# argsim/argsim

Hardware: AMD Instinct MI355X
Metric: sentences/sec per ELBO step (higher is better)
Workload: dtype f32; 1 GPU; BASELINE configs[1]: 1xMI355X fp32, latent_dim 128, vocab 8k, seq_len 64, batch 256 per GPU; FULL synthetic Zipf batches, dim_emb 512, 3 layers, step 20000; global_batch=256, seq_len=64, parallelism=dp1, gru=persistent

## Files before the change

### argsim_amd/csrc/gemm_f32.hip

```cpp
#include "kernels.h"
#include "mfma_tile.h"
#include <algorithm>
#include <cstdlib>
#include <type_traits>

namespace avae {

constexpr int BK = kTileBK, LDK = kTileLDK;

template <bool XC, int ROWS>
struct FastTile {
    const float* base; long long step, valid; unsigned voff[ROWS / 32];
    __device__ __forceinline__ void init(const float* P, int ld, int x0, int X, int kb, int ke, int tid)
    {
        if (XC) {
            base = P + (size_t)kb * ld + x0; step = (long long)BK * ld; valid = (long long)(ke - kb) * ld - x0;
#pragma unroll
            for (int rep = 0; rep < ROWS / 32; ++rep) { const int f = tid + 256 * rep; voff[rep] = (unsigned)(((f / (ROWS / 4)) * ld + ((f % (ROWS / 4)) << 2)) * 4); }
        } else {
            base = P + (size_t)x0 * ld + kb; step = BK; valid = (long long)(X - x0) * ld - kb;
#pragma unroll
            for (int rep = 0; rep < ROWS / 32; ++rep) { const int f = tid + 256 * rep; voff[rep] = (unsigned)(((f >> 3) * ld + ((f & 7) << 2)) * 4); }
        }
    }
    __device__ __forceinline__ void load(float4 (&r)[ROWS / 32], int it) const
    {
        const long long rem = valid - it * step;
        const unsigned bytes = rem <= 0 ? 0u : (rem >= (1ll << 30) ? 0xFFFFFFFFu : (unsigned)(rem * 4));
        const __amdgpu_buffer_rsrc_t rs = __builtin_amdgcn_make_buffer_rsrc(const_cast<float*>(base + it * step), 0, (int)bytes, 0x00020000);
#pragma unroll
        for (int rep = 0; rep < ROWS / 32; ++rep) {
            const u32x4 v = __builtin_amdgcn_raw_buffer_load_b128(rs, (int)voff[rep], 0, 0);
            r[rep] = make_float4(__uint_as_float(v.x), __uint_as_float(v.y), __uint_as_float(v.z), __uint_as_float(v.w));
        }
    }
};

template <int MODE>
__device__ __forceinline__ void put(float* c, float v)
{
    if (MODE == 2) atomicAdd(c, v);
    else if (MODE == 1) *c += v;
    else *c = v;
}
template <int TM, int TN, int WN, int MODE>
__device__ __forceinline__ void epilogue_full(const GemmArgs& g, const f32x16 (&acc)[TM][TN], int m0, int n0, int wm, int wn, int h, int l31, bool add_bias)
{
    float bv[TN];
#pragma unroll
    for (int j = 0; j < TN; ++j) bv[j] = add_bias ? g.bias[n0 + 32 * (wn * TN + j) + l31] : 0.f;
#pragma unroll
    for (int j = 0; j < TN; ++j) {
        const int col = n0 + 32 * (wn * TN + j) + l31;
#pragma unroll
        for (int i = 0; i < TM; ++i) {
            float* c = g.C + (size_t)(m0 + 32 * (wm * TM + i) + 4 * h) * g.ldc + col;
#pragma unroll
            for (int r = 0; r < 16; ++r)
                put<MODE>(c + (size_t)mfma32_row(r, 0) * g.ldc, g.alpha * acc[i][j][r] + bv[j]);
        }
    }
}
template <int TM, int TN, int WN>
__device__ __forceinline__ void epilogue(const GemmArgs& g, const f32x16 (&acc)[TM][TN], int M, int m0, int n0, int BM, int BN,
                                         int wm, int wn, int h, int l31, bool atomic, bool add_bias)
{
    if (!atomic && m0 + BM <= M && n0 + BN <= g.N) {
        if (g.accumulate) epilogue_full<TM, TN, WN, 1>(g, acc, m0, n0, wm, wn, h, l31, add_bias);
        else epilogue_full<TM, TN, WN, 0>(g, acc, m0, n0, wm, wn, h, l31, add_bias);
        return;
    }
    epilogue_generic<TM, TN>(acc, g.C, g.ldc, M, g.N, m0 + 32 * wm * TM, n0 + 32 * wn * TN, h, l31, g.alpha, add_bias ? g.bias : nullptr,
                             atomic ? kEpiAtomic : (g.accumulate ? kEpiAccumulate : kEpiStore));
}

template <bool A_MC, bool B_NC, int WM, int WN, int TM, int TN, bool FAST = false, bool DB = false>
__global__ __launch_bounds__(256, DB ? 2 : 3) void gemm_f32_kernel(GemmArgs g)
{
    constexpr int BM = 32 * WM * TM, BN = 32 * WN * TN;
    constexpr int kStage = (BM + BN) * LDK;
    __shared__ __attribute__((aligned(16))) float smem[kStage * (DB ? 2 : 1)];
    float* As = smem;
    float* Bs = smem + BM * LDK;

    const int tid = threadIdx.x, lane = tid & 63, wave = tid >> 6;
    const int h = lane >> 5, l31 = lane & 31;
    const int wm = wave / WN, wn = wave % WN;

    if (blockIdx.y) { g.A = g.A2; g.B = g.B2; g.C = g.C2; g.bias = g.bias2; }
    int M = g.M, K = g.K;
    if (g.dyn_kind == 1) M = min(M, *g.dyn);
    if (g.dyn_kind == 2) K = min(K, *g.dyn);

    const int tiles_n = (g.N + BN - 1) / BN;
    const int nblk = ((M + BM - 1) / BM) * tiles_n;
    const int bid = xcd_tile(blockIdx.x, nblk);
    if (bid < 0) return;
    const int tm = bid / tiles_n, tn = bid - tm * tiles_n;
    const int m0 = tm * BM, n0 = tn * BN;
    if (m0 >= M) return;

    int kb = 0, ke = K;
    if (g.split_k > 1) {
        int ktiles = (K + BK - 1) / BK;
        int per = (ktiles + g.split_k - 1) / g.split_k;
        kb = blockIdx.z * per * BK;
        ke = min(K, kb + per * BK);
        if (kb >= ke) return;
    }

    f32x16 acc[TM][TN];
    zero_acc(acc);

    float4 ra[BM / 32], rb[BN / 32];
    FastTile<A_MC, BM> fa; FastTile<B_NC, BN> fb;
    if (FAST) {
        fa.init(g.A, g.lda, m0, M, kb, ke, tid); fb.init(g.B, g.ldb, n0, g.N, kb, ke, tid);
        fa.load(ra, 0); fb.load(rb, 0);
    } else {
        load_tile<A_MC, BM>(ra, g.A, g.lda, m0, M, kb, ke, tid);
        load_tile<B_NC, BN>(rb, g.B, g.ldb, n0, g.N, kb, ke, tid);
    }

    if (DB) {
        store_tile<A_MC, BM>(As, ra, tid);
        store_tile<B_NC, BN>(Bs, rb, tid);
        __syncthreads();
    }
    for (int k0 = kb; k0 < ke; k0 += BK) {
        auto next_loads = [&]() __attribute__((always_inline)) {
            if (k0 + BK < ke) {
                if (FAST) { const int it = (k0 - kb) / BK + 1; fa.load(ra, it); fb.load(rb, it); }
                else {
                    load_tile<A_MC, BM>(ra, g.A, g.lda, m0, M, k0 + BK, ke, tid);
                    load_tile<B_NC, BN>(rb, g.B, g.ldb, n0, g.N, k0 + BK, ke, tid);
                }
            }
        };
        if (!DB) {
            store_tile<A_MC, BM>(As, ra, tid);
            store_tile<B_NC, BN>(Bs, rb, tid);
            next_loads();
            __syncthreads();
        } else next_loads();
        __builtin_amdgcn_s_setprio(1);
#pragma unroll
        for (int q = 0; q < 4; ++q) {
            float a[TM][4], b[TN][4];
#pragma unroll
            for (int t = 0; t < TM; ++t) {
                if (A_MC) {
#pragma unroll
                    for (int e = 0; e < 4; ++e) a[t][e] = As[(8 * q + 4 * h + e) * BM + 32 * (wm * TM + t) + l31];
                } else {
                    float4 v = *reinterpret_cast<const float4*>(As + (32 * (wm * TM + t) + l31) * LDK + 8 * q + 4 * h);
                    a[t][0] = v.x; a[t][1] = v.y; a[t][2] = v.z; a[t][3] = v.w;
                }
            }
#pragma unroll
            for (int t = 0; t < TN; ++t) {
                if (B_NC) {
#pragma unroll
                    for (int e = 0; e < 4; ++e) b[t][e] = Bs[(8 * q + 4 * h + e) * BN + 32 * (wn * TN + t) + l31];
                } else {
                    float4 v = *reinterpret_cast<const float4*>(Bs + (32 * (wn * TN + t) + l31) * LDK + 8 * q + 4 * h);
                    b[t][0] = v.x; b[t][1] = v.y; b[t][2] = v.z; b[t][3] = v.w;
                }
            }
#pragma unroll
            for (int e = 0; e < 4; ++e)
#pragma unroll
                for (int i = 0; i < TM; ++i)
#pragma unroll
                    for (int j = 0; j < TN; ++j)
                        acc[i][j] = __builtin_amdgcn_mfma_f32_32x32x2f32(a[i][e], b[j][e], acc[i][j], 0, 0, 0);
        }
        __builtin_amdgcn_s_setprio(0);
        if (DB) {
            As = (As == smem) ? smem + kStage : smem;
            Bs = As + BM * LDK;
            if (k0 + BK < ke) {
                store_tile<A_MC, BM>(As, ra, tid);
                store_tile<B_NC, BN>(Bs, rb, tid);
            }
        }
        __syncthreads();
    }

    const bool atomic = g.split_k > 1;
    const bool add_bias = g.bias != nullptr && (!atomic || blockIdx.z == 0);
    epilogue<TM, TN, WN>(g, acc, M, m0, n0, BM, BN, wm, wn, h, l31, atomic, add_bias);
}

template <bool A_MC, bool B_NC, bool FAST>
__global__ __launch_bounds__(256, 3) void gemm_f32_persist_kernel(GemmArgs g)
{
    static_assert(FAST, "buffer-load staging only (register budget of three workgroups per CU)");
    constexpr int TM = 2, TN = 2, WN = 2, BM = 128, BN = 128;
    __shared__ __attribute__((aligned(16))) float smem[(BM + BN) * LDK];
    float* As = smem;
    float* Bs = smem + BM * LDK;
    const int tid = threadIdx.x, lane = tid & 63, wave = tid >> 6;
    const int h = lane >> 5, l31 = lane & 31;
    const int wm = wave / WN, wn = wave % WN;

    int M = g.M;
    const int K = g.K;
    if (g.dyn_kind == 1) M = min(M, *g.dyn);
    const int tiles_n = (g.N + BN - 1) / BN;
    const int nblk = ((M + BM - 1) / BM) * tiles_n;
    const int per_xcd = gridDim.x >> 3;
    int run0, run_n;
    xcd_run(blockIdx.x & 7, nblk, run0, run_n);
    int local = blockIdx.x >> 3;
    if (local >= run_n) return;

    float4 ra[BM / 32], rb[BN / 32];
    FastTile<A_MC, BM> fa; FastTile<B_NC, BN> fb;
    auto first_tile = [&](int bid) __attribute__((always_inline)) {
        const int tm = bid / tiles_n, tn = bid - tm * tiles_n;
        if (FAST) {
            fa.init(g.A, g.lda, tm * BM, M, 0, K, tid); fb.init(g.B, g.ldb, tn * BN, g.N, 0, K, tid);
            fa.load(ra, 0); fb.load(rb, 0);
        } else {
            load_tile<A_MC, BM>(ra, g.A, g.lda, tm * BM, M, 0, K, tid);
            load_tile<B_NC, BN>(rb, g.B, g.ldb, tn * BN, g.N, 0, K, tid);
        }
    };
    first_tile(run0 + local);
    for (; local < run_n; local += per_xcd) {
        const int bid = run0 + local;
        const int tm = bid / tiles_n, tn = bid - tm * tiles_n;
        const int m0 = tm * BM, n0 = tn * BN;
        const bool more = local + per_xcd < run_n;
        f32x16 acc[TM][TN];
        zero_acc(acc);
        for (int k0 = 0; k0 < K; k0 += BK) {
            store_tile<A_MC, BM>(As, ra, tid);
            store_tile<B_NC, BN>(Bs, rb, tid);
// ... 45 lines not shown
                } else b[u] = *reinterpret_cast<const float4*>(bp + k);
            }
        }
#pragma unroll
        for (int u = 0; u < 4; ++u) {
            if (kk + 8 * u >= k1) break;
            acc = __builtin_amdgcn_mfma_f32_32x32x2f32(a[u].x, b[u].x, acc, 0, 0, 0);
            acc = __builtin_amdgcn_mfma_f32_32x32x2f32(a[u].y, b[u].y, acc, 0, 0, 0);
            acc = __builtin_amdgcn_mfma_f32_32x32x2f32(a[u].z, b[u].z, acc, 0, 0, 0);
            acc = __builtin_amdgcn_mfma_f32_32x32x2f32(a[u].w, b[u].w, acc, 0, 0, 0);
        }
    }
    if (wave > 0) {
#pragma unroll
        for (int r = 0; r < 16; ++r) red[wave - 1][r][lane] = acc[r];
    }
    __syncthreads();
    if (wave > 0) return;
    const int col = n0 + l31;
    if (col >= g.N) return;
    const float bv = g.bias ? g.bias[col] : 0.f;
#pragma unroll
    for (int r = 0; r < 16; ++r) {
        float v = acc[r];
#pragma unroll
        for (int w = 0; w < 7; ++w) v += red[w][r][lane];
        const int row = m0 + mfma32_row(r, h);
        if (row >= g.M) continue;
        float* c = g.C + (size_t)row * g.ldc + col;
        v = g.alpha * v + bv;
        if (g.accumulate) *c += v; else *c = v;
    }
}
static bool skinny_ok(bool a_mc, const GemmArgs& g)
{
    return !a_mc && g.split_k <= 1 && g.dyn_kind == 0 && (g.K & 3) == 0 && (g.lda & 3) == 0 && g.K >= 64;
}
static void launch_skinny(hipStream_t st, bool b_nc, const GemmArgs& g, const GemmF32Form& f)
{
    const dim3 grid(f.gx, f.gy, f.gz);
    if (b_nc) hipLaunchKernelGGL(gemm_f32_skinny_kernel<true>, grid, dim3(512), 0, st, g);
    else      hipLaunchKernelGGL(gemm_f32_skinny_kernel<false>, grid, dim3(512), 0, st, g);
}

template <class F>
static void with_layouts(bool a_mc, bool b_nc, F&& f)
{
    if (!a_mc && !b_nc)      f(std::false_type{}, std::false_type{});
    else if (!a_mc && b_nc)  f(std::false_type{}, std::true_type{});
    else if (a_mc && b_nc)   f(std::true_type{}, std::true_type{});
    else                     f(std::true_type{}, std::false_type{});
}

GemmF32Form gemm_f32_form(bool a_mc, bool b_nc, const GemmArgs& g)
{
    GemmF32Form f{-1, false, false, false, 0, 0, 0, hipSuccess};
    if (g.M <= 0 || g.N <= 0) return f;
    f.err = hipErrorInvalidValue;
    if ((g.lda | g.ldb) & 3) return f;
    if (((uintptr_t)g.A | (uintptr_t)g.B | (uintptr_t)g.A2 | (uintptr_t)g.B2) & 15) return f;
    if (!a_mc && (g.K & 3)) return f;
    if (a_mc && (g.M & 3)) return f;
    if (!b_nc && (g.K & 3)) return f;
    if (b_nc && (g.N & 3)) return f;
    if (g.dyn_kind == 2 && (!a_mc || !b_nc || (g.split_k > 1 && g.bias))) return f;
    f.err = hipSuccess;
    if (g.thin == 3 && skinny_ok(a_mc, g) && (b_nc || (g.ldb & 3) == 0)) {
        f.tile = 3; f.gx = ((g.M + 31) / 32) * ((g.N + 31) / 32); f.gy = g.A2 ? 2 : 1; f.gz = 1;
        return f;
    }
    f.tile = g.thin == 2 ? 2 : (g.thin ? 1 : 0);
    const int BM = f.tile == 0 ? 128 : (f.tile == 1 ? 32 : 64), BN = f.tile == 2 ? 64 : 128;
    const int tiles = ((g.M + BM - 1) / BM) * ((g.N + BN - 1) / BN);
    f.gx = tiles; f.gy = g.A2 ? 2 : 1; f.gz = g.split_k > 1 ? g.split_k : 1;
    static const bool allow_fast = !getenv("AVAE_F32_NOFAST");
    const int k_per_wg = g.split_k > 1 ? (g.K + g.split_k - 1) / g.split_k : g.K;
    f.fast = allow_fast && (a_mc ? (g.M % BM == 0) : (g.K % BK == 0 && g.dyn_kind != 2)) &&
             (b_nc ? (g.N % BN == 0) : (g.K % BK == 0 && g.dyn_kind != 2)) && (a_mc || b_nc || k_per_wg >= 1536);
    if (f.tile == 1) return f;
    static const char* ps_env = getenv("AVAE_F32_PERSIST");
    const bool aligned = (a_mc ? (g.M % BM == 0) : (g.K % BK == 0)) && (b_nc ? (g.N % BN == 0) : (g.K % BK == 0));
    const bool persist = (ps_env ? atoi(ps_env) != 0 : true) && allow_fast && aligned && !g.A2 && g.split_k <= 1 && g.dyn_kind != 2 && tiles > 1024;
    if (persist) {
        f.tile = 0; f.fast = true; f.persist = true; f.gx = 768; f.gy = f.gz = 1;
        return f;
    }
    static const char* db_env = getenv("AVAE_F32_DB");
    const int eff_tiles = (g.dyn_kind == 1 && g.dyn_expect > 0) ? std::min(tiles, ((g.dyn_expect + BM - 1) / BM) * ((g.N + BN - 1) / BN)) : (g.dyn_kind == 1 ? 0 : tiles);
    f.db = db_env ? atoi(db_env) != 0 && !g.A2 : (!g.A2 && g.split_k <= 1 && eff_tiles > 768 && tiles <= 1024);
    return f;
}

template <int WM, int WN, int TM, int TN>
static void launch_variant(hipStream_t st, bool a_mc, bool b_nc, const GemmArgs& g, const GemmF32Form& f)
{
    const dim3 grid(f.gx, f.gy, f.gz);
    if constexpr (WM == 2 && WN == 2) {
        if (f.persist) {
            with_layouts(a_mc, b_nc, [&](auto A, auto B) { hipLaunchKernelGGL((gemm_f32_persist_kernel<decltype(A)::value, decltype(B)::value, true>), grid, dim3(256), 0, st, g); });
            return;
        }
        if (f.db) {
            if (f.fast) {
                with_layouts(a_mc, b_nc, [&](auto A, auto B) { hipLaunchKernelGGL((gemm_f32_kernel<decltype(A)::value, decltype(B)::value, WM, WN, TM, TN, true, true>), grid, dim3(256), 0, st, g); });
            } else {
                with_layouts(a_mc, b_nc, [&](auto A, auto B) { hipLaunchKernelGGL((gemm_f32_kernel<decltype(A)::value, decltype(B)::value, WM, WN, TM, TN, false, true>), grid, dim3(256), 0, st, g); });
            }
            return;
        }
    }
    if (f.fast) {
        with_layouts(a_mc, b_nc, [&](auto A, auto B) { hipLaunchKernelGGL((gemm_f32_kernel<decltype(A)::value, decltype(B)::value, WM, WN, TM, TN, true>), grid, dim3(256), 0, st, g); });
        return;
    }
    with_layouts(a_mc, b_nc, [&](auto A, auto B) { hipLaunchKernelGGL((gemm_f32_kernel<decltype(A)::value, decltype(B)::value, WM, WN, TM, TN>), grid, dim3(256), 0, st, g); });
}

hipError_t gemm_f32(hipStream_t st, bool a_mc, bool b_nc, const GemmArgs& g)
{
    const GemmF32Form f = gemm_f32_form(a_mc, b_nc, g);
    if (f.err != hipSuccess) return f.err;
    if (f.tile < 0) return hipSuccess;
    if (f.tile == 3) launch_skinny(st, b_nc, g, f);
    else if (f.persist) launch_variant<2, 2, 2, 2>(st, a_mc, b_nc, g, f);
    else if (f.tile == 2) launch_variant<2, 2, 1, 1>(st, a_mc, b_nc, g, f);
    else if (f.tile == 1) launch_variant<1, 4, 1, 1>(st, a_mc, b_nc, g, f);
    else launch_variant<2, 2, 2, 2>(st, a_mc, b_nc, g, f);
    return hipGetLastError();
}

}
```

### argsim_amd/csrc/handle.cpp

```cpp
#include "ctx.h"

using namespace avae;
using namespace avae::host;

static std::string g_create_err;

namespace avae { namespace host {

int grow_scratch(avae_ctx* h, size_t need, const char* what)
{
    if (h->scratch_n >= (int64_t)need) return 0;
    AV_CHECK(hipStreamSynchronize(h->stream));
    if (h->scratch) AV_CHECK(hipFree(h->scratch));
    h->scratch = nullptr; h->scratch_n = 0;
    if (hipMalloc(reinterpret_cast<void**>(&h->scratch), need) != hipSuccess) {
        (void)hipGetLastError();
        h->scratch = nullptr;
        char b_[256]; snprintf(b_, sizeof b_, "%s: %.0f MB of scratch could not be allocated on the device", what, (double)need / 1048576.0);
        return fail(h, b_);
    }
    h->scratch_n = (int64_t)need;
    return 0;
}

// ... 178 lines not shown
    if (shape) for (int i = 0; i < 4; ++i) shape[i] = e->shape[i];
    return 0;
}

static int xfer_tensor(avae_handle h, const char* name, int kind, float* buf, bool get)
{
    if (!h) return 1;
    AV_TRY(check_bound(h));
    const ParamEntry* e = find_param(h, name);
    if (!e) return fail(h, std::string("unknown variable: ") + (name ? name : "(null)"));
    float* base = state_buf(h, kind);
    if (!base) return fail(h, "bad tensor kind");
    float* flat = base + e->offset;
    int64_t n = e->shape[0] * e->shape[1] * e->shape[2] * e->shape[3];
    if (!e->g16) {
        AV_CHECK(hipMemcpyAsync(get ? buf : flat, get ? flat : buf, n * sizeof(float), hipMemcpyDeviceToDevice, h->stream));
    } else {
        int D = h->cfg.dim_emb, cols = (int)(e->ndim == 2 ? e->shape[1] : 1);
        if (get) AV_CHECK(g16_permute(h->stream, buf, flat, D, cols, false));
        else     AV_CHECK(g16_permute(h->stream, flat, buf, D, cols, true));
    }
    return 0;
}
int avae_get_tensor(avae_handle h, const char* name, int kind, float* buf) { return xfer_tensor(h, name, kind, buf, true); }
int avae_set_tensor(avae_handle h, const char* name, int kind, const float* buf) { return xfer_tensor(h, name, kind, const_cast<float*>(buf), false); }

int avae_get_step(avae_handle h, int64_t* s) { if (!h || !s) return 1; *s = h->step; return 0; }
int avae_set_step(avae_handle h, int64_t s) { if (!h) return 1; h->step = s; return 0; }

int avae_set_grad_hook(avae_handle h, avae_grad_hook hook, void* user) { if (!h) return 1; h->hook = hook; h->hook_user = user; return 0; }

int avae_set_option(avae_handle h, const char* key, int value)
{
    if (!h || !key) return 1;
    if (!strcmp(key, "persistent")) { h->persistent = value; return 0; }
    if (!strcmp(key, "gru_item")) { h->gru_item = value; return 0; }
    if (!strcmp(key, "gru_stagger")) { h->gru_stagger = value; return 0; }
    if (!strcmp(key, "gru_force_slow")) { h->gru_force_slow = value; return 0; }
    if (!strcmp(key, "gru_bf16")) { h->gru_bf16 = value != 0; return 0; }
    if (!strcmp(key, "bwd_rs")) { h->bwd_rs = value; return 0; }
    if (!strcmp(key, "dyn_split")) { h->dyn_split = value != 0; return 0; }
    if (!strcmp(key, "shared_device")) { h->shared_device = value != 0; return 0; }
    if (!strcmp(key, "gru_spec")) { h->gru_spec = value; return 0; }
    if (!strcmp(key, "gru_ring")) { h->gru_ring = value != 0; return 0; }
    if (!strcmp(key, "bf16_nt8")) { h->bf16_nt8 = value != 0; return 0; }
    if (!strcmp(key, "logits16")) { h->logits16 = value != 0; return 0; }
    if (!strcmp(key, "bf16_direct")) { h->bf16_direct = value != 0; return 0; }
    if (!strcmp(key, "bf16_tn")) { h->bf16_tn = value != 0; return 0; }
    if (!strcmp(key, "bf16_sv")) { h->bf16_sv = value != 0; return 0; }
    if (!strcmp(key, "bf16_act")) { h->bf16_act = value != 0; return 0; }
    if (!strcmp(key, "table_l1")) { h->table_l1 = value != 0; return 0; }
    if (!strcmp(key, "enc_top1")) { h->enc_top1 = value != 0; return 0; }
    if (!strcmp(key, "dyn_thin")) { h->dyn_thin = value != 0; return 0; }
    if (!strcmp(key, "skip_pad")) { h->skip_pad = value != 0; return 0; }
    if (!strcmp(key, "compact")) { h->compact = value; return 0; }
    if (!strcmp(key, "skinny")) { h->skinny = value; return 0; }
    if (!strcmp(key, "knn_chunk")) { if (value < 0) return fail(h, "knn_chunk must be >= 0"); h->knn_chunk = value; return 0; }
    if (!strcmp(key, "agg_chunk")) { if (value < 0) return fail(h, "agg_chunk must be >= 0"); h->agg_chunk = value; return 0; }
    if (!strcmp(key, "ward_form")) { if (value < 0 || value > 2) return fail(h, "ward_form must be 0 (planner), 1 (one-workgroup) or 2 (launch-per-merge)"); h->ward_form = value; return 0; }
    if (!strcmp(key, "probe_chunk")) { if (value < 0) return fail(h, "probe_chunk must be >= 0"); h->probe_chunk = value; return 0; }
    if (!strcmp(key, "kmeans_chunk")) { if (value < 0) return fail(h, "kmeans_chunk must be >= 0"); h->kmeans_chunk = value; return 0; }
    if (!strcmp(key, "tsne_chunk")) { if (value < 0) return fail(h, "tsne_chunk must be >= 0"); h->tsne_chunk = value; return 0; }
    if (!strcmp(key, "gru_ablate")) {
        if (value && !gru_diag_build()) return fail(h, "gru_ablate needs the diagnostic build of libargsim_vae.so (make -C argsim_amd/csrc DIAG=1)");
        h->gru_ablate = value; return 0;
    }
    if (!strcmp(key, "timing")) { h->timing = value; h->timing_on = value; h->stamps_used = 0; return 0; }
    if (!strcmp(key, "timing_pause")) { h->timing = value ? 0 : h->timing_on; return 0; }
    return fail(h, "unknown option");
}
int avae_timing_collect(avae_handle h, double* out)
{
    if (!h || !out) return 1;
    AV_CHECK(hipStreamSynchronize(h->stream));
    for (int i = 0; i < 9; ++i) out[i] = 0.0;
    std::vector<std::pair<const int*, int>> seen;
    for (size_t i = 0; i < h->stamps_used; ++i) {
        float ms = 0.f;
        AV_CHECK(hipEventElapsedTime(&ms, h->stamps[i].a, h->stamps[i].b));
        double f = 1.0;
        AV_TRY(dyn_fraction(h, h->stamps[i], seen, &f));
        int c = h->stamps[i].cls;
        out[3 * c] += ms; out[3 * c + 1] += 1.0; out[3 * c + 2] += h->stamps[i].flops * f;
    }
    h->stamps_used = 0;
    return 0;
}
int avae_bucket_count(avae_handle h) { return h ? (int)h->buckets.size() : 0; }
int avae_bucket_info(avae_handle h, int i, int64_t* offset, int64_t* count)
{
    if (!h || i < 0 || i >= (int)h->buckets.size()) return 1;
    *offset = h->buckets[i].first; *count = h->buckets[i].second; return 0;
}

}
```

### argsim_amd/csrc/hooks.cpp

```cpp
#include "ctx.h"

using namespace avae;
using namespace avae::host;

extern "C" {

int avae_debug_team_batch(int32_t B) { return B > 0 ? gru_team_batch(B) : 0; }
int avae_debug_gemm_plan(const int32_t* in, int32_t n, int32_t* out)
{
    if (!in || !out || n < 0) return 1;
    for (int r = 0; r < n; ++r, in += 19, out += 15) {
        const GemmShape s{in[0] != 0, in[1] != 0, in[2], in[3], in[4], in[5], in[6], in[7], in[8], in[9], in[10], in[11] != 0, in[12] != 0,
                          in[13] != 0, in[14] != 0, in[15], in[16] != 0, in[17] != 0, in[18] != 0};
        const GemmPlan p = gemm_plan(s);
        out[0] = p.n;
        for (int i = 0; i < 2; ++i) {
            const GemmLaunch l = i < p.n ? p.launch[i] : GemmLaunch{0, 0, 0, 0, 0, 0, 0};
            const int32_t f[7] = {l.row0, l.rows, l.thin, l.split_k, l.accumulate, l.zero, l.dyn};
            std::copy(f, f + 7, out + 1 + 7 * i);
        }
    }
    return 0;
}
int avae_debug_gemm_call(avae_handle h, int a_mc, int b_nc, const float* A, const float* Bm, float* Cm, const float* bias, int M, int N, int K,
                         int lda, int ldb, int ldc, float alpha, int accumulate, int flags, const int* count, int expect,
                         const float* A2, const float* B2, float* C2, unsigned short* keep16)
{
    if (!h) return 1;
    GemmCall c{A, lda, a_mc != 0, Bm, ldb, b_nc != 0, Cm, ldc, M, N, K};
    c.alpha = alpha; c.bias = bias; c.accumulate = accumulate; c.keep_a16 = keep16;
    c.allow_atomic = (flags & 1) != 0; c.rows_are_batch = (flags & 2) != 0; c.wgrad = (flags & 4) != 0;
    if (c.wgrad) c.depth(count); else c.rows(count);
    const Pair second{A2, B2, C2, nullptr};
    if (A2) c.pair = &second;
    const int* const was_ptr = h->expect_ptr[0]; const int was_val = h->expect_val[0];
    h->expect_ptr[0] = count; h->expect_val[0] = expect;
    const int r = gemm(h, c);
    h->expect_ptr[0] = was_ptr; h->expect_val[0] = was_val;
    return r;
}
int avae_debug_gemm_forced(avae_handle h, int a_mc, int b_nc, const float* A, const float* Bm, float* Cm, const float* bias, int M, int N, int K,
                           int lda, int ldb, int ldc, float alpha, int accumulate, int thin, int split_k, const int* count, int dyn_kind, int expect,
                           const float* A2, const float* B2, float* C2, const float* bias2)
{
    if (!h) return 1;
    if (thin < 0 || thin > 3 || split_k < 1 || dyn_kind < 0 || dyn_kind > 2 || (dyn_kind != 0) != (count != nullptr))
        return fail(h, "avae_debug_gemm_forced: thin in 0..3, split_k >= 1, dyn_kind in 0..2 with a count exactly where it is not 0");
    GemmCall c{A, lda, a_mc != 0, Bm, ldb, b_nc != 0, Cm, ldc, M, N, K};
    c.alpha = alpha; c.bias = bias; c.accumulate = accumulate;
    if (dyn_kind == 2) c.depth(count); else c.rows(count);
    c.form(thin, split_k);
    const Pair second{A2, B2, C2, bias2};
    if (A2) c.pair = &second;
    const int* const was_ptr = h->expect_ptr[0]; const int was_val = h->expect_val[0];
    h->expect_ptr[0] = count; h->expect_val[0] = expect;
    const int r = gemm(h, c);
    h->expect_ptr[0] = was_ptr; h->expect_val[0] = was_val;
    return r;
}
int avae_debug_gemm_f32_form(int a_mc, int b_nc, int M, int N, int K, int lda, int ldb, int ldc, int accumulate, int thin, int split_k, int dyn_kind,
                             int expect, int pair, int32_t out[8])
{
    if (!out) return 1;
    alignas(16) static const float other[4] = {0.f, 0.f, 0.f, 0.f};
    const GemmArgs g{nullptr, nullptr, nullptr, nullptr, M, N, K, lda, ldb, ldc, 1.f, accumulate, split_k, nullptr, dyn_kind, expect, thin,
                     pair ? other : nullptr, pair ? other : nullptr, nullptr, nullptr};
    const GemmF32Form f = gemm_f32_form(a_mc != 0, b_nc != 0, g);
    const int32_t v[8] = {f.tile, f.fast, f.db, f.persist, (int32_t)f.gx, (int32_t)f.gy, (int32_t)f.gz, f.err != hipSuccess};
    std::copy(v, v + 8, out);
    return 0;
}
int avae_debug_score_plan(avae_handle h, int32_t out[4])
{
    if (!h || !out) return 1;
    for (int i = 0; i < 4; ++i) out[i] = h->score_plan[i];
    return 0;
}
int avae_debug_present_ids(avae_handle h, int32_t out[2])
{
    if (!h || !out) return 1;
    AV_CHECK(hipStreamSynchronize(h->stream));
    out[0] = out[1] = -1;
    if (h->cnt_src) AV_CHECK(hipMemcpy(&out[0], h->cnt_src, sizeof(int), hipMemcpyDeviceToHost));
    if (h->cnt_tgt) AV_CHECK(hipMemcpy(&out[1], h->cnt_tgt, sizeof(int), hipMemcpyDeviceToHost));
    return 0;
}
int avae_debug_train_ce(avae_handle h, float* out, int32_t max_n, int32_t* n_out)
{
    if (!h || !out || !n_out) return 1;
    if (h->B < 1) return fail(h, "avae_debug_train_ce: no training forward has run on this handle");
    Ws w;
    AV_TRY(get_ws(h, w, h->B, h->Ss, h->St, true));
    int n = 0;
    AV_CHECK(hipMemcpyAsync(&n, w.ntok, sizeof(int), hipMemcpyDeviceToHost, h->stream));
    AV_CHECK(hipStreamSynchronize(h->stream));
    n = std::min(n, (int)max_n);
    AV_CHECK(hipMemcpyAsync(out, w.loss_samp, (size_t)n * sizeof(float), hipMemcpyDeviceToDevice, h->stream));
    *n_out = n;
    return 0;
}
int avae_debug_timing(avae_handle h, double* out, int max_n, int* n)
{
    if (!h || !out || !n) return 1;
    AV_CHECK(hipStreamSynchronize(h->stream));
    *n = (int)std::min<size_t>(h->stamps_used, (size_t)max_n);
    std::vector<std::pair<const int*, int>> seen;
    for (int i = 0; i < *n; ++i) {
        float ms = 0.f;
        AV_CHECK(hipEventElapsedTime(&ms, h->stamps[i].a, h->stamps[i].b));
        double f = 1.0;
        AV_TRY(dyn_fraction(h, h->stamps[i], seen, &f));
        const double fl = h->stamps[i].flops * f;
        out[3 * i] = h->stamps[i].cls; out[3 * i + 1] = ms; out[3 * i + 2] = fl;
    }
    return 0;
}
int avae_debug_stamps(avae_handle h, unsigned long long* out)
{
    if (!h || !out) return 1;
    AV_CHECK(hipStreamSynchronize(h->stream));
    AV_CHECK(hipMemcpy(out, h->errw + 16, 32 * sizeof(unsigned long long), hipMemcpyDeviceToHost));
    AV_CHECK(hipMemset(h->errw + 16, 0, 32 * sizeof(unsigned long long)));
    return 0;
// ... 219 lines not shown
```

### argsim_amd/csrc/kernels.h

```cpp
#pragma once
#include <hip/hip_runtime.h>
#include <stdint.h>

#include "gemm_plan.h"

namespace avae {

struct GemmArgs {
    const float* A; const float* B; float* C; const float* bias;
    int M, N, K, lda, ldb, ldc;
    float alpha;
    int accumulate;
    int split_k;
    const int* dyn; int dyn_kind;
    int dyn_expect;
    int thin;
    const float* A2; const float* B2; float* C2; const float* bias2;
    float* slab = nullptr; size_t slab_floats = 0;
    unsigned short* c16 = nullptr;
    int nt8 = 1;
};
hipError_t gemm_f32(hipStream_t st, bool a_mc, bool b_nc, const GemmArgs& g);
struct GemmF32Form { int tile; bool fast, db, persist; unsigned gx, gy, gz; hipError_t err; };
GemmF32Form gemm_f32_form(bool a_mc, bool b_nc, const GemmArgs& g);
hipError_t gemm_f32s(hipStream_t st, bool a_mc, bool b_nc, const GemmArgs& g);
hipError_t gemm_bf16_direct(hipStream_t st, bool a_mc, bool b_nc, const GemmArgs& g);

hipError_t cvt_bf16(hipStream_t st, const float* src, int ld, bool transpose, int rows_or_K, int cols_or_X,
                    unsigned short* dst, int ldd);
hipError_t gemm_bf16_nt(hipStream_t st, const unsigned short* A, int lda, const unsigned short* B, int ldb, const GemmArgs& g);
bool gemm_bf16_p8_ok(const GemmArgs& g, int lda, int ldb);
hipError_t gemm_bf16_p8(hipStream_t st, const unsigned short* A, int lda, const unsigned short* B, int ldb, const GemmArgs& g, int s2);
bool gemm_bf16_c16_ok(const GemmArgs& g, int lda, int ldb);
bool gemm_bf16_c16_takes(int M, int N, int K, const int* rows, int nt8);
bool gemm_bf16_p8_tn_ok(const GemmArgs& g, int lda, int ldb);
hipError_t gemm_bf16_p8_tn(hipStream_t st, const unsigned short* A, int lda, const unsigned short* B, int ldb, const GemmArgs& g, int s2);
hipError_t gemm_bf16_tn(hipStream_t st, const unsigned short* A, int lda, const unsigned short* B, int ldb, const GemmArgs& g);
hipError_t transpose_bf16(hipStream_t st, const unsigned short* src, int ld, int K, int X, unsigned short* dst, int ldk);

constexpr int kMaxGruJobs = 3;
struct GruJob {
    const float* gi;
    const int32_t* gi_rows;
    const float* R;
    const float* bR;
    const float* h0;
    float* hs;
    float* sv;
    float* hp;
    int reverse;
    unsigned short* hs16;
    unsigned short* hp16;
    const float* dh_out;
    float* dgi;
    float* dgh;
    unsigned short* dgi16;
    unsigned short* dgh16;
    float* dh0;
    float* carry;
    int dgi_by_pos;
    float* dbW;
    float* dbR;
};
struct GruArgs {
    GruJob job[kMaxGruJobs];
    int njobs, S, B, D, ldg, ldh;
    const int* lens;
    const int* slens;
    const int* perm;
    const int* rowmap;
    int Bx;
    int G;
    int rows_per_group;
    int p_begin, p_end;
    unsigned* counters;
    int* err;
    unsigned long long* stamps;
// ... 351 lines not shown
```

### argsim_amd/lib.py

```python
import ctypes as C
import os
import subprocess

_HERE = os.path.dirname(os.path.abspath(__file__))
LIB_PATH = os.path.join(_HERE, 'libargsim_vae.so')
CSRC = os.path.join(_HERE, 'csrc')


def source_digest():
    import glob
    import hashlib
    h = hashlib.sha1()
    files = sorted(glob.glob(os.path.join(CSRC, '*.hip')) + glob.glob(os.path.join(CSRC, '*.cpp')) + glob.glob(os.path.join(CSRC, '*.h')))
    files.append(os.path.join(os.path.dirname(_HERE), 'include', 'argsim_vae.h'))
    for f in files:
        h.update(os.path.basename(f).encode())
        with open(f, 'rb') as fh:
            h.update(fh.read())
    return h.hexdigest()[:16]


class AvaeConfig(C.Structure):
    _fields_ = [('dim_tgt', C.c_int32), ('dim_emb', C.c_int32), ('dim_rep', C.c_int32), ('rnn_layers', C.c_int32),
                ('accelerate', C.c_float), ('learn_rate', C.c_float), ('bos', C.c_int32), ('eos', C.c_int32),
# ... 75 lines not shown
    'avae_get_step': (C.c_int, [_P, C.POINTER(C.c_int64)]),
    'avae_set_step': (C.c_int, [_P, C.c_int64]),
    'avae_get_schedule': (C.c_int, [_P, C.POINTER(C.c_float)]),
    'avae_forward_backward': (C.c_int, [_P, _P, _P, C.c_int32, C.c_int32, C.c_int32, C.c_uint64, _P, _P, C.c_float, C.c_float]),
    'avae_adam_step': (C.c_int, [_P]),
    'avae_train_step': (C.c_int, [_P, _P, _P, C.c_int32, C.c_int32, C.c_int32, C.c_uint64, _P, _P]),
    'avae_get_losses': (C.c_int, [_P, C.POINTER(C.c_float)]),
    'avae_set_grad_hook': (C.c_int, [_P, GRAD_HOOK, _P]),
    'avae_eval': (C.c_int, [_P, _P, _P, C.c_int32, C.c_int32, C.c_int32, _P, _P, _P, C.POINTER(C.c_int32)]),
    'avae_encode': (C.c_int, [_P, _P, C.c_int32, C.c_int32, _P, _P]),
    'avae_decode_init': (C.c_int, [_P, _P, C.c_int32, _P]),
    'avae_decode_step': (C.c_int, [_P, _P, _P, C.c_int32, _P, _P]),
    'avae_decode_greedy': (C.c_int, [_P, _P, C.c_int32, C.c_int32, _P, C.POINTER(C.c_int32)]),
    'avae_decode_sample': (C.c_int, [_P, _P, C.c_int32, C.c_int32, C.POINTER(AvaeSampleConfig), _P, _P, C.POINTER(C.c_int32)]),
    'avae_decode_sample_p': (C.c_int, [_P, _P, C.c_int32, C.c_int32, C.POINTER(AvaeSamplePConfig), _P, _P, _P, C.POINTER(C.c_int32)]),
    'avae_decode_beam': (C.c_int, [_P, _P, C.c_int32, C.c_int32, C.POINTER(AvaeBeamConfig), _P, _P, _P, _P, _P, _P, _P, C.POINTER(C.c_int32)]),
    'avae_score': (C.c_int, [_P, _P, _P, C.c_int32, C.c_int32, C.c_int32, C.POINTER(AvaeScoreConfig), _P, _P, _P, _P, _P, _P]),
    'avae_score_z': (C.c_int, [_P, _P, _P, C.c_int32, C.c_int32, _P, _P]),
    'avae_knn': (C.c_int, [_P, _P, C.c_int32, _P, C.c_int32, C.c_int32, C.POINTER(AvaeKnnConfig), _P, _P]),
    'avae_agg_logq': (C.c_int, [_P, _P, C.c_int32, _P, _P, C.c_int32, C.c_int32, C.POINTER(AvaeAggConfig), _P, _P]),
    'avae_latent_moments': (C.c_int, [_P, _P, _P, C.c_int32, C.c_int32, _P]),
    'avae_probe_fit': (C.c_int, [_P, _P, C.c_int32, C.c_int32, _P, C.c_int32, C.POINTER(AvaeProbeConfig), _P, _P]),
    'avae_probe_decision': (C.c_int, [_P, _P, C.c_int32, C.c_int32, _P, C.c_int32, _P]),
    'avae_probe_fit_l1': (C.c_int, [_P, _P, C.c_int32, C.c_int32, _P, C.c_int32, C.POINTER(AvaeProbeL1Config), _P, _P]),
    'avae_ward': (C.c_int, [_P, _P, C.c_int32, C.POINTER(C.c_int32), C.c_int32, C.POINTER(AvaeWardConfig), _P, _P, _P]),
    'avae_ward_cut': (C.c_int, [_P, _P, C.POINTER(C.c_int32), C.c_int32, C.POINTER(C.c_int32), _P]),
    'avae_affinity': (C.c_int, [_P, _P, C.c_int32, C.c_int32, C.POINTER(AvaeAffinityConfig), _P, _P, _P, _P, _P]),
    'avae_tsne': (C.c_int, [_P, _P, C.c_int32, C.c_int32, C.POINTER(AvaeTsneConfig)] + [_P] * 10),
    'avae_kmeans': (C.c_int, [_P, _P, C.c_int32, C.c_int32, C.POINTER(AvaeKmeansConfig)] + [_P] * 8),
    'avae_set_option': (C.c_int, [_P, C.c_char_p, C.c_int]),
    'avae_debug_gemm': (C.c_int, [_P, C.c_int, C.c_int, _P, _P, _P, _P] + [C.c_int] * 6 + [C.c_float, C.c_int, C.c_int]),
    'avae_debug_gemm_dyn': (C.c_int, [_P, _P, _P, _P, C.c_int, C.c_int, C.c_int, _P]),
    'avae_debug_gemm_c16': (C.c_int, [_P, _P, _P, _P, C.c_int, C.c_int, C.c_int, C.c_float, _P]),
    'avae_debug_gemm_tn16': (C.c_int, [_P, _P, _P, _P] + [C.c_int] * 6 + [C.c_float]),
    'avae_debug_softmax_ce': (C.c_int, [_P, _P, _P, C.c_int, _P, _P, _P, C.c_int, C.c_int, C.c_int, C.c_float, _P, _P, _P, C.POINTER(C.c_int)]),
    'avae_debug_argmax_rows': (C.c_int, [_P, _P, _P, C.c_int, C.c_int]),
    'avae_debug_op': (C.c_int, [_P, C.c_char_p, C.POINTER(_P), C.POINTER(C.c_int64), C.POINTER(C.c_float)]),
    'avae_debug_op_layout': (C.c_int, [C.c_int64, C.c_int64, C.POINTER(C.c_int64)]),
    'avae_debug_sample_rows': (C.c_int, [_P, _P, C.c_int, C.c_int, C.c_int, C.POINTER(AvaeSampleConfig), _P, _P]),
    'avae_debug_sample_rows_p': (C.c_int, [_P, _P, C.c_int, C.c_int, C.c_int, C.POINTER(AvaeSamplePConfig), _P, _P, _P, _P]),
    'avae_debug_beam_select': (C.c_int, [_P, _P, C.c_int, C.c_int, C.c_int, _P, _P, _P, _P, _P, _P]),
    'avae_timing_collect': (C.c_int, [_P, C.POINTER(C.c_double)]),
    'avae_debug_timing': (C.c_int, [_P, C.POINTER(C.c_double), C.c_int, C.POINTER(C.c_int)]),
    'avae_debug_train_ce': (C.c_int, [_P, _P, C.c_int32, C.POINTER(C.c_int32)]),
    'avae_debug_stamps': (C.c_int, [_P, C.POINTER(C.c_uint64)]),
    'avae_debug_present_ids': (C.c_int, [_P, C.POINTER(C.c_int32)]),
    'avae_debug_score_plan': (C.c_int, [_P, C.POINTER(C.c_int32)]),
    'avae_debug_team_batch': (C.c_int, [C.c_int32]),
    'avae_debug_gemm_plan': (C.c_int, [_P, C.c_int32, _P]),
    'avae_debug_gemm_call': (C.c_int, [_P, C.c_int, C.c_int, _P, _P, _P, _P] + [C.c_int] * 6 + [C.c_float, C.c_int, C.c_int, _P, C.c_int, _P, _P, _P, _P]),
    'avae_debug_gemm_forced': (C.c_int, [_P, C.c_int, C.c_int, _P, _P, _P, _P] + [C.c_int] * 6 + [C.c_float, C.c_int, C.c_int, C.c_int, _P, C.c_int, C.c_int,
                                         _P, _P, _P, _P]),
    'avae_debug_gemm_f32_form': (C.c_int, [C.c_int] * 14 + [C.POINTER(C.c_int32)]),
    'avae_debug_gru_plan': (C.c_int, [C.POINTER(C.c_int64), C.c_int, C.c_int, C.POINTER(C.c_int64)]),
    'avae_debug_gru': (C.c_int, [_P, C.c_int, C.c_int, C.POINTER(C.c_int64), C.POINTER(_P), C.POINTER(_P), C.POINTER(C.c_int64)]),
    'avae_bucket_count': (C.c_int, [_P]),
    'avae_bucket_info': (C.c_int, [_P, C.c_int, C.POINTER(C.c_int64), C.POINTER(C.c_int64)]),
}

_lib = None


def build(force=False, jobs=4):
    if force:
        subprocess.run(['make', '-C', CSRC, 'clean'], check=True, stdout=subprocess.DEVNULL)
    subprocess.run(['make', '-C', CSRC, '-j%d' % jobs], check=True, stdout=subprocess.DEVNULL)
    return LIB_PATH


def load():
    global _lib
    if _lib is not None:
        return _lib
    if not os.path.exists(LIB_PATH):
        raise RuntimeError("libargsim_vae.so is not built: run `python -c 'import __graft_entry__ as g; g.build()'` "
                           "(there is no CPU fallback for the HIP path)")
    lib = C.CDLL(LIB_PATH)
    for name, (res, args) in SIGNATURES.items():
        fn = getattr(lib, name)
        fn.restype = res
        fn.argtypes = args
    _lib = lib
    return lib
```

Measured before the change: 15950 sentences/sec.

## Keep two k-tiles of global loads in flight in f32 GEMM kernel

Adds a D2 variant of the f32 MFMA GEMM kernel that holds two sets of register staging buffers, so loads for tile k+2 are issued while tile k is stored and computed, deepening global-load prefetch without a second LDS stage. It is enabled by default for the tile-2 form when both operands are [k][x] layout, buffer-load staging is used and double-buffering is off. It is selectable via env var or a handle knob. This costs more VGPRs, which could reduce occupancy under the 3-workgroup launch bound, and adds an extra barrier per tile.

```diff
diff --git a/argsim_amd/csrc/gemm_f32.hip b/argsim_amd/csrc/gemm_f32.hip
--- a/argsim_amd/csrc/gemm_f32.hip
+++ b/argsim_amd/csrc/gemm_f32.hip
@@ -74,9 +74,10 @@
                              atomic ? kEpiAtomic : (g.accumulate ? kEpiAccumulate : kEpiStore));
 }
 
-template <bool A_MC, bool B_NC, int WM, int WN, int TM, int TN, bool FAST = false, bool DB = false>
+template <bool A_MC, bool B_NC, int WM, int WN, int TM, int TN, bool FAST = false, bool DB = false, bool D2 = false>
 __global__ __launch_bounds__(256, DB ? 2 : 3) void gemm_f32_kernel(GemmArgs g)
 {
+    static_assert(!D2 || (FAST && A_MC && B_NC && !DB), "two tiles in flight: [k][x] operands, buffer-load staging, single LDS stage");
     constexpr int BM = 32 * WM * TM, BN = 32 * WN * TN;
     constexpr int kStage = (BM + BN) * LDK;
     __shared__ __attribute__((aligned(16))) float smem[kStage * (DB ? 2 : 1)];
@@ -112,79 +113,118 @@
     f32x16 acc[TM][TN];
     zero_acc(acc);
 
-    float4 ra[BM / 32], rb[BN / 32];
-    FastTile<A_MC, BM> fa; FastTile<B_NC, BN> fb;
-    if (FAST) {
+    if constexpr (D2) {
+        float4 ra0[BM / 32], rb0[BN / 32], ra1[BM / 32], rb1[BN / 32];
+        FastTile<A_MC, BM> fa; FastTile<B_NC, BN> fb;
         fa.init(g.A, g.lda, m0, M, kb, ke, tid); fb.init(g.B, g.ldb, n0, g.N, kb, ke, tid);
-        fa.load(ra, 0); fb.load(rb, 0);
+        const int nt = (ke - kb + BK - 1) / BK;
+        fa.load(ra0, 0); fb.load(rb0, 0);
+        fa.load(ra1, 1); fb.load(rb1, 1);
+        auto burst = [&](int wm, int wn, int h, int l31) __attribute__((always_inline)) {
+            __syncthreads();
+            __builtin_amdgcn_s_setprio(1);
+            mfma_ktile<A_MC, B_NC, TM, TN, BM, BN>(acc, As, Bs, wm, wn, h, l31);
+            __builtin_amdgcn_s_setprio(0);
+            __syncthreads();
+        };
+        int it = 0;
+        for (; it + 2 <= nt; it += 2) {
+            store_tile<A_MC, BM>(As, ra0, tid);
+            store_tile<B_NC, BN>(Bs, rb0, tid);
+            fa.load(ra0, it + 2); fb.load(rb0, it + 2);
+            burst(wm, wn, h, l31);
+            store_tile<A_MC, BM>(As, ra1, tid);
+            store_tile<B_NC, BN>(Bs, rb1, tid);
+            fa.load(ra1, it + 3); fb.load(rb1, it + 3);
+            burst(wm, wn, h, l31);
+        }
+        int t2 = tid;
+        asm volatile("" : "+v"(t2));
+        const int wm2 = (t2 >> 6) / WN, wn2 = (t2 >> 6) % WN, h2 = (t2 & 63) >> 5, l2 = t2 & 31;
+        if (it < nt) {
+            store_tile<A_MC, BM>(As, ra0, t2);
+            store_tile<B_NC, BN>(Bs, rb0, t2);
+            burst(wm2, wn2, h2, l2);
+        }
+        const bool atomic = g.split_k > 1;
+        const bool add_bias = g.bias != nullptr && (!atomic || blockIdx.z == 0);
+        epilogue<TM, TN, WN>(g, acc, M, m0, n0, BM, BN, wm2, wn2, h2, l2, atomic, add_bias);
+        return;
     } else {
-        load_tile<A_MC, BM>(ra, g.A, g.lda, m0, M, kb, ke, tid);
-        load_tile<B_NC, BN>(rb, g.B, g.ldb, n0, g.N, kb, ke, tid);
-    }
-
-    if (DB) {
-        store_tile<A_MC, BM>(As, ra, tid);
-        store_tile<B_NC, BN>(Bs, rb, tid);
-        __syncthreads();
-    }
-    for (int k0 = kb; k0 < ke; k0 += BK) {
-        auto next_loads = [&]() __attribute__((always_inline)) {
-            if (k0 + BK < ke) {
-                if (FAST) { const int it = (k0 - kb) / BK + 1; fa.load(ra, it); fb.load(rb, it); }
-                else {
-                    load_tile<A_MC, BM>(ra, g.A, g.lda, m0, M, k0 + BK, ke, tid);
-                    load_tile<B_NC, BN>(rb, g.B, g.ldb, n0, g.N, k0 + BK, ke, tid);
+        float4 ra[BM / 32], rb[BN / 32];
+        FastTile<A_MC, BM> fa; FastTile<B_NC, BN> fb;
+        if (FAST) {
+            fa.init(g.A, g.lda, m0, M, kb, ke, tid); fb.init(g.B, g.ldb, n0, g.N, kb, ke, tid);
+            fa.load(ra, 0); fb.load(rb, 0);
+        } else {
+            load_tile<A_MC, BM>(ra, g.A, g.lda, m0, M, kb, ke, tid);
+            load_tile<B_NC, BN>(rb, g.B, g.ldb, n0, g.N, kb, ke, tid);
+        }
+
+        if (DB) {
+            store_tile<A_MC, BM>(As, ra, tid);
+            store_tile<B_NC, BN>(Bs, rb, tid);
+            __syncthreads();
+        }
+        for (int k0 = kb; k0 < ke; k0 += BK) {
+            auto next_loads = [&]() __attribute__((always_inline)) {
+                if (k0 + BK < ke) {
+                    if (FAST) { const int it = (k0 - kb) / BK + 1; fa.load(ra, it); fb.load(rb, it); }
+                    else {
+                        load_tile<A_MC, BM>(ra, g.A, g.lda, m0, M, k0 + BK, ke, tid);
+                        load_tile<B_NC, BN>(rb, g.B, g.ldb, n0, g.N, k0 + BK, ke, tid);
+                    }
+                }
+            };
+            if (!DB) {
+                store_tile<A_MC, BM>(As, ra, tid);
+                store_tile<B_NC, BN>(Bs, rb, tid);
+                next_loads();
+                __syncthreads();
+            } else next_loads();
+            __builtin_amdgcn_s_setprio(1);
+    #pragma unroll
+            for (int q = 0; q < 4; ++q) {
+                float a[TM][4], b[TN][4];
+    #pragma unroll
+                for (int t = 0; t < TM; ++t) {
+                    if (A_MC) {
+    #pragma unroll
+                        for (int e = 0; e < 4; ++e) a[t][e] = As[(8 * q + 4 * h + e) * BM + 32 * (wm * TM + t) + l31];
+                    } else {
+                        float4 v = *reinterpret_cast<const float4*>(As + (32 * (wm * TM + t) + l31) * LDK + 8 * q + 4 * h);
+                        a[t][0] = v.x; a[t][1] = v.y; a[t][2] = v.z; a[t][3] = v.w;
+                    }
+                }
+    #pragma unroll
+                for (int t = 0; t < TN; ++t) {
+                    if (B_NC) {
+    #pragma unroll
+                        for (int e = 0; e < 4; ++e) b[t][e] = Bs[(8 * q + 4 * h + e) * BN + 32 * (wn * TN + t) + l31];
+                    } else {
+                        float4 v = *reinterpret_cast<const float4*>(Bs + (32 * (wn * TN + t) + l31) * LDK + 8 * q + 4 * h);
+                        b[t][0] = v.x; b[t][1] = v.y; b[t][2] = v.z; b[t][3] = v.w;
+                    }
+                }
+    #pragma unroll
+                for (int e = 0; e < 4; ++e)
+    #pragma unroll
+                    for (int i = 0; i < TM; ++i)
+    #pragma unroll
+                        for (int j = 0; j < TN; ++j)
+                            acc[i][j] = __builtin_amdgcn_mfma_f32_32x32x2f32(a[i][e], b[j][e], acc[i][j], 0, 0, 0);
+            }
+            __builtin_amdgcn_s_setprio(0);
+            if (DB) {
+                As = (As == smem) ? smem + kStage : smem;
+                Bs = As + BM * LDK;
+                if (k0 + BK < ke) {
+                    store_tile<A_MC, BM>(As, ra, tid);
+                    store_tile<B_NC, BN>(Bs, rb, tid);
                 }
             }
-        };
-        if (!DB) {
-            store_tile<A_MC, BM>(As, ra, tid);
-            store_tile<B_NC, BN>(Bs, rb, tid);
-            next_loads();
-            __syncthreads();
-        } else next_loads();
-        __builtin_amdgcn_s_setprio(1);
-#pragma unroll
-        for (int q = 0; q < 4; ++q) {
-            float a[TM][4], b[TN][4];
-#pragma unroll
-            for (int t = 0; t < TM; ++t) {
-                if (A_MC) {
-#pragma unroll
-                    for (int e = 0; e < 4; ++e) a[t][e] = As[(8 * q + 4 * h + e) * BM + 32 * (wm * TM + t) + l31];
-                } else {
-                    float4 v = *reinterpret_cast<const float4*>(As + (32 * (wm * TM + t) + l31) * LDK + 8 * q + 4 * h);
-                    a[t][0] = v.x; a[t][1] = v.y; a[t][2] = v.z; a[t][3] = v.w;
-                }
-            }
-#pragma unroll
-            for (int t = 0; t < TN; ++t) {
-                if (B_NC) {
-#pragma unroll
-                    for (int e = 0; e < 4; ++e) b[t][e] = Bs[(8 * q + 4 * h + e) * BN + 32 * (wn * TN + t) + l31];
-                } else {
-                    float4 v = *reinterpret_cast<const float4*>(Bs + (32 * (wn * TN + t) + l31) * LDK + 8 * q + 4 * h);
-                    b[t][0] = v.x; b[t][1] = v.y; b[t][2] = v.z; b[t][3] = v.w;
-                }
-            }
-#pragma unroll
-            for (int e = 0; e < 4; ++e)
-#pragma unroll
-                for (int i = 0; i < TM; ++i)
-#pragma unroll
-                    for (int j = 0; j < TN; ++j)
-                        acc[i][j] = __builtin_amdgcn_mfma_f32_32x32x2f32(a[i][e], b[j][e], acc[i][j], 0, 0, 0);
-        }
-        __builtin_amdgcn_s_setprio(0);
-        if (DB) {
-            As = (As == smem) ? smem + kStage : smem;
-            Bs = As + BM * LDK;
-            if (k0 + BK < ke) {
-                store_tile<A_MC, BM>(As, ra, tid);
-                store_tile<B_NC, BN>(Bs, rb, tid);
-            }
-        }
-        __syncthreads();
+            __syncthreads();
+        }
     }
 
     const bool atomic = g.split_k > 1;
@@ -336,9 +376,12 @@
     else                     f(std::true_type{}, std::false_type{});
 }
 
+constexpr int kDepth2Forms = 1;
+static int depth2_override = -1;
+void gemm_f32_depth2_forms(int forms) { depth2_override = forms; }
 GemmF32Form gemm_f32_form(bool a_mc, bool b_nc, const GemmArgs& g)
 {
-    GemmF32Form f{-1, false, false, false, 0, 0, 0, hipSuccess};
+    GemmF32Form f{-1, false, false, false, 0, 0, 0, hipSuccess, false};
     if (g.M <= 0 || g.N <= 0) return f;
     f.err = hipErrorInvalidValue;
     if ((g.lda | g.ldb) & 3) return f;
@@ -372,6 +415,9 @@
     static const char* db_env = getenv("AVAE_F32_DB");
     const int eff_tiles = (g.dyn_kind == 1 && g.dyn_expect > 0) ? std::min(tiles, ((g.dyn_expect + BM - 1) / BM) * ((g.N + BN - 1) / BN)) : (g.dyn_kind == 1 ? 0 : tiles);
     f.db = db_env ? atoi(db_env) != 0 && !g.A2 : (!g.A2 && g.split_k <= 1 && eff_tiles > 768 && tiles <= 1024);
+    static const char* d2_env = getenv("AVAE_F32_DEPTH2");
+    const int d2 = depth2_override >= 0 ? depth2_override : (d2_env ? atoi(d2_env) : kDepth2Forms);
+    f.depth2 = f.fast && !f.db && a_mc && b_nc && (((f.tile == 2 ? d2 : d2 >> 1) & 1) != 0);
     return f;
 }
 
@@ -380,6 +426,10 @@
 {
     const dim3 grid(f.gx, f.gy, f.gz);
     if constexpr (WM == 2 && WN == 2) {
+        if (f.depth2) {
+            hipLaunchKernelGGL((gemm_f32_kernel<true, true, WM, WN, TM, TN, true, false, true>), grid, dim3(256), 0, st, g);
+            return;
+        }
         if (f.persist) {
             with_layouts(a_mc, b_nc, [&](auto A, auto B) { hipLaunchKernelGGL((gemm_f32_persist_kernel<decltype(A)::value, decltype(B)::value, true>), grid, dim3(256), 0, st, g); });
             return;
diff --git a/argsim_amd/csrc/handle.cpp b/argsim_amd/csrc/handle.cpp
--- a/argsim_amd/csrc/handle.cpp
+++ b/argsim_amd/csrc/handle.cpp
@@ -254,6 +254,7 @@
     if (!strcmp(key, "table_l1")) { h->table_l1 = value != 0; return 0; }
     if (!strcmp(key, "enc_top1")) { h->enc_top1 = value != 0; return 0; }
     if (!strcmp(key, "dyn_thin")) { h->dyn_thin = value != 0; return 0; }
+    if (!strcmp(key, "f32_depth2")) { gemm_f32_depth2_forms(value); return 0; }
     if (!strcmp(key, "skip_pad")) { h->skip_pad = value != 0; return 0; }
     if (!strcmp(key, "compact")) { h->compact = value; return 0; }
     if (!strcmp(key, "skinny")) { h->skinny = value; return 0; }
diff --git a/argsim_amd/csrc/hooks.cpp b/argsim_amd/csrc/hooks.cpp
--- a/argsim_amd/csrc/hooks.cpp
+++ b/argsim_amd/csrc/hooks.cpp
@@ -69,6 +69,15 @@
     const int32_t v[8] = {f.tile, f.fast, f.db, f.persist, (int32_t)f.gx, (int32_t)f.gy, (int32_t)f.gz, f.err != hipSuccess};
     std::copy(v, v + 8, out);
     return 0;
+}
+int avae_debug_gemm_f32_depth2(int a_mc, int b_nc, int M, int N, int K, int lda, int ldb, int ldc, int accumulate, int thin, int split_k, int dyn_kind,
+                               int expect, int pair)
+{
+    alignas(16) static const float other[4] = {0.f, 0.f, 0.f, 0.f};
+    const GemmArgs g{nullptr, nullptr, nullptr, nullptr, M, N, K, lda, ldb, ldc, 1.f, accumulate, split_k, nullptr, dyn_kind, expect, thin,
+                     pair ? other : nullptr, pair ? other : nullptr, nullptr, nullptr};
+    const GemmF32Form f = gemm_f32_form(a_mc != 0, b_nc != 0, g);
+    return (f.tile < 0 || f.err != hipSuccess) ? -1 : (f.depth2 ? 1 : 0);
 }
 int avae_debug_score_plan(avae_handle h, int32_t out[4])
 {
diff --git a/argsim_amd/csrc/kernels.h b/argsim_amd/csrc/kernels.h
--- a/argsim_amd/csrc/kernels.h
+++ b/argsim_amd/csrc/kernels.h
@@ -21,8 +21,9 @@
     int nt8 = 1;
 };
 hipError_t gemm_f32(hipStream_t st, bool a_mc, bool b_nc, const GemmArgs& g);
-struct GemmF32Form { int tile; bool fast, db, persist; unsigned gx, gy, gz; hipError_t err; };
+struct GemmF32Form { int tile; bool fast, db, persist; unsigned gx, gy, gz; hipError_t err; bool depth2; };
 GemmF32Form gemm_f32_form(bool a_mc, bool b_nc, const GemmArgs& g);
+void gemm_f32_depth2_forms(int forms);
 hipError_t gemm_f32s(hipStream_t st, bool a_mc, bool b_nc, const GemmArgs& g);
 hipError_t gemm_bf16_direct(hipStream_t st, bool a_mc, bool b_nc, const GemmArgs& g);
 
diff --git a/argsim_amd/lib.py b/argsim_amd/lib.py
--- a/argsim_amd/lib.py
+++ b/argsim_amd/lib.py
@@ -151,6 +151,7 @@
     'avae_debug_gemm_forced': (C.c_int, [_P, C.c_int, C.c_int, _P, _P, _P, _P] + [C.c_int] * 6 + [C.c_float, C.c_int, C.c_int, C.c_int, _P, C.c_int, C.c_int,
                                          _P, _P, _P, _P]),
     'avae_debug_gemm_f32_form': (C.c_int, [C.c_int] * 14 + [C.POINTER(C.c_int32)]),
+    'avae_debug_gemm_f32_depth2': (C.c_int, [C.c_int] * 14),
     'avae_debug_gru_plan': (C.c_int, [C.POINTER(C.c_int64), C.c_int, C.c_int, C.POINTER(C.c_int64)]),
     'avae_debug_gru': (C.c_int, [_P, C.c_int, C.c_int, C.POINTER(C.c_int64), C.POINTER(_P), C.POINTER(_P), C.POINTER(C.c_int64)]),
     'avae_bucket_count': (C.c_int, [_P]),
```

After: 16010 sentences/sec, median of 6. About the same (+0.4%).
